# LuoGroup2023/PanTax

Hardware: AMD Instinct MI355X
Metric: PAO wall-time (s) + Mreads/s: packed reads + DB (graphs and their unique-trio index) resident in HBM -> abundance tables; the metric's own GAF -> abundance quantity is value_gaf_to_tables (files -> tables, never `value`) (higher is better)
Workload: dtype int64+f64

## Files before the change

### pantax_amd/csrc/cov_device.hpp

```cpp
#pragma once
#include "common.hpp"
#include "wave.hpp"

namespace ptx {

constexpr int COV_BLOCK = 256;

__device__ __forceinline__ uint32_t bm_peek(const uint32_t *p) {
    return __hip_atomic_load(p, __ATOMIC_RELAXED, __HIP_MEMORY_SCOPE_AGENT);
}
constexpr uint32_t COV_BWIN = 2048;
constexpr int COV_WIN = 2048;
extern __shared__ uint32_t s_cov[];
#define S_WIN(i) s_cov[(i)]
#define S_BM(bmo, i) s_cov[(bmo) + (i)]
#define S_FULL(bmo, i) reinterpret_cast<uint8_t *>(s_cov + (bmo) + COV_BWIN)[(i)]
__host__ __device__ constexpr size_t cov_lds_bytes(int win) { return (size_t)win * 4 + COV_BWIN * 4 + (size_t)win; }
__device__ __forceinline__ void lds_or(uint32_t *__restrict__ bm, uint32_t bmo, uint64_t bw0, uint32_t bwn, uint64_t w, uint32_t m) {
    const uint64_t off = w - bw0;
    if (off < bwn) {
        if ((S_BM(bmo, off) & m) != m) atomicOr(&S_BM(bmo, off), m);
    } else if ((bm_peek(&bm[w]) & m) != m) atomicOr(&bm[w], m);
}
__device__ __forceinline__ void mark_range(uint32_t *__restrict__ bm, uint32_t bmo, uint64_t bw0, uint32_t bwn, uint64_t g0, uint64_t g1) {
    if (g1 <= g0) return;
    uint64_t w0 = g0 >> 5, w1 = (g1 - 1) >> 5;
    uint32_t m0 = 0xFFFFFFFFu << (g0 & 31);
    uint32_t m1 = 0xFFFFFFFFu >> (31 - (uint32_t)((g1 - 1) & 31));
    if (w0 == w1) lds_or(bm, bmo, bw0, bwn, w0, m0 & m1);
    else {
        lds_or(bm, bmo, bw0, bwn, w0, m0);
        for (uint64_t w = w0 + 1; w < w1; ++w) lds_or(bm, bmo, bw0, bwn, w, 0xFFFFFFFFu);
        lds_or(bm, bmo, bw0, bwn, w1, m1);
    }
}
__device__ __forceinline__ void win_or(uint32_t bmo, uint32_t w, uint32_t m) { if ((S_BM(bmo, w) & m) != m) atomicOr(&S_BM(bmo, w), m); }
__device__ __forceinline__ void mark_window(uint32_t bmo, uint32_t r0, uint32_t r1) {
    if (r1 <= r0) return;
    const uint32_t w0 = r0 >> 5, w1 = (r1 - 1) >> 5;
    const uint32_t m0 = 0xFFFFFFFFu << (r0 & 31), m1 = 0xFFFFFFFFu >> (31 - ((r1 - 1) & 31));
    if (w0 == w1) win_or(bmo, w0, m0 & m1);
    else {
        win_or(bmo, w0, m0);
        for (uint32_t w = w0 + 1; w < w1; ++w) win_or(bmo, w, 0xFFFFFFFFu);
        win_or(bmo, w1, m1);
    }
}

constexpr uint32_t STEP_LONG = 0x80u;
constexpr uint32_t STEP_START = 0x40u, STEP_PAD = 0xFFu, STEP_DIST = 0x3Fu;
__device__ __forceinline__ unsigned long long ballot1(bool b) { return __builtin_amdgcn_ballot_w64(b); }
__device__ __forceinline__ bool any1(bool b) { return __builtin_amdgcn_ballot_w64(b) != 0ull; }
__device__ __forceinline__ bool none1(bool b) { return __builtin_amdgcn_ballot_w64(b) == 0ull; }
__device__ __forceinline__ uint32_t slot_in_group(uint32_t group_first_slot, uint32_t code, int lane) {
    const unsigned long long starts = ballot1((code != STEP_PAD) & ((code & STEP_START) != 0u)) & ~1ull;
    const uint32_t below = __builtin_amdgcn_mbcnt_hi((uint32_t)(starts >> 32), __builtin_amdgcn_mbcnt_lo((uint32_t)starts, 0u));
    return group_first_slot + below + (uint32_t)((starts >> lane) & 1ull);
}

__device__ __forceinline__ uint32_t rl_from_memory(uint32_t j, uint32_t b, const uint32_t *__restrict__ node_id, const uint8_t *__restrict__ step_dup,
                                                   uint32_t delta, const uint4 *__restrict__ node_rec, uint32_t len0, uint32_t ps) {
    const uint32_t idj = node_id[b + j];
    if (j == 0 || ((step_dup[b + j] & 1u) && idj == node_id[b])) return len0 - ps;
    return node_rec[idj + delta].z;
}

#ifdef COV_ABLATE
#define ABL(bit) (ablate & (bit))
#else
#define ABL(bit) false
#endif
constexpr int COV_WIN_BACK = 128;
constexpr uint32_t NO_SLOT = 0xFFFFFFFFu;

__device__ __forceinline__ void add_bases(unsigned long long *__restrict__ bases, uint32_t wlo, uint32_t win_n, uint32_t v, uint32_t aln) {
    const uint32_t off = v - wlo;
    if (off < win_n && aln < (1u << 18)) atomicAdd(&S_WIN(off), aln);
    else atomicAdd(&bases[v], (unsigned long long)aln);
}
constexpr uint32_t NO_FULL = 0xFFFFFFFFu;
__device__ __forceinline__ void mark_full_wave(uint32_t *__restrict__ full, uint32_t wlo, uint32_t win_n, uint32_t v) {
    const uint32_t off = v - wlo;
    const bool have = v != NO_FULL;
    if (have && off < win_n) S_FULL(COV_WIN, off) = 1;
    const bool out = have && off >= win_n;
    unsigned long long todo = __ballot(out);
    const uint32_t w = v >> 5, bit = 1u << (v & 31);
    const int lane = threadIdx.x & 63;
    while (todo) {
        const int leader = __builtin_ctzll(todo);
        const uint32_t wl = (uint32_t)__builtin_amdgcn_readlane((int)w, leader);
        const bool mine = out && w == wl;
        const uint32_t orv = wave_reduce(mine ? bit : 0u, [](uint32_t x, uint32_t y) { return x | y; });
        if (lane == leader) atomicOr(&full[wl], orv);
        todo &= ~__ballot(mine);
    }
}

constexpr uint32_t COV_ITEM_GROUPS = 128;
struct __attribute__((packed, aligned(4))) EntPair { uint32_t a, b, c, d; };
constexpr int COV_BLK_SHIFT = 11;

template <int WIN>
__device__ __forceinline__ void mark_full_out_wave(uint32_t *__restrict__ full, bool out, uint32_t v) {
    unsigned long long todo = ballot1(out);
    const uint32_t w = v >> 5, bit = 1u << (v & 31);
    const int lane = threadIdx.x & 63;
    while (todo) {
        const int leader = __builtin_ctzll(todo);
        const uint32_t wl = (uint32_t)__builtin_amdgcn_readlane((int)w, leader);
        const bool mine = out & (w == wl);
        const uint32_t orv = wave_reduce(mine ? bit : 0u, [](uint32_t x, uint32_t y) { return x | y; });
        if (lane == leader) atomicOr(&full[wl], orv);
        todo &= ~ballot1(mine);
    }
}

}
```

### pantax_amd/csrc/stage_cov.hip

```cpp
#include <chrono>
#include <cstdio>
#include <cstdlib>
#include "common.hpp"
#include "primitives.hpp"
#include "wave.hpp"
#include "cov_plan.hpp"
#include "cov_device.hpp"
#pragma clang diagnostic ignored "-Wbitwise-instead-of-logical"

namespace ptx {

template <bool WITH_TRIO, int U, int PASSES, int WIN, bool LONG = false>
#if !defined(COV_NO_PF3) && !defined(COV_NO_PF2) && !defined(COV_NO_PREFETCH)
__attribute__((amdgpu_waves_per_eu((U <= 2 && !LONG) ? 6 : 1)))
#endif
__global__ void __launch_bounds__(COV_BLOCK) coverage_fast_kernel(
    const uint2 *__restrict__ items, const uint32_t *__restrict__ group_slot, const uint4 *__restrict__ read_rec, const uint2 *__restrict__ slot_rec,
    const uint32_t *__restrict__ node_id, const uint8_t *__restrict__ step_code, const uint8_t *__restrict__ active,
    const uint4 *__restrict__ node_rec, const uint64_t *__restrict__ bit_off, uint64_t V, unsigned long long *__restrict__ bases,
    uint32_t *__restrict__ bitmap, uint32_t *__restrict__ full, const uint2 *__restrict__ trio_ent, unsigned long long *__restrict__ trio_bases,
    unsigned long long *__restrict__ n_abort, uint32_t ablate, int blk_shift,
    const uint32_t *__restrict__ long_sum = nullptr, const uint32_t *__restrict__ long_len0 = nullptr, uint32_t only_long = 0u,
    uint32_t chunk_groups = 0u, uint32_t total_groups = 0u, uint32_t win_back = 0u, const uint32_t *__restrict__ item_sel = nullptr,
    uint32_t spec_miss = 0u) {
    constexpr int WAVES = COV_BLOCK / 64;
#if !defined(COV_NO_PF3) && !defined(COV_NO_PF2) && !defined(COV_NO_PREFETCH)
    const int lane = threadIdx.x & 63, wave = LONG ? (int)(threadIdx.x >> 6) : __builtin_amdgcn_readfirstlane((int)(threadIdx.x >> 6));
#else
    const int lane = threadIdx.x & 63, wave = threadIdx.x >> 6;
#endif
    uint32_t g0, n_groups;
    if constexpr (LONG) { g0 = blockIdx.x * chunk_groups; n_groups = min(g0 + chunk_groups, total_groups); }
    else { const uint2 item = items[item_sel ? item_sel[blockIdx.x] : blockIdx.x]; g0 = item.x; n_groups = item.y; }
    for (int i = threadIdx.x; i < (int)(cov_lds_bytes(WIN) / 4); i += COV_BLOCK) s_cov[i] = 0;
    uint32_t wlo = 0, win_n = 0, mark_n = 0, bit0_lo = 0, bwn = 0;
    uint64_t bw0 = 0;
    uint32_t s0 = 0xFFFFFFFFu, dlt0 = 0;
#pragma unroll 1
    for (uint32_t g = g0; g < n_groups && win_n == 0; ++g) {
        const uint32_t gs = group_slot[g];
        if (gs == NO_SLOT) continue;
        const uint2 sr0 = slot_rec[gs];
        if ((int)sr0.x < 0 || !active[sr0.x]) continue;
        s0 = sr0.x; dlt0 = sr0.y;
        const uint32_t id0 = node_id[(uint64_t)g * 64], v0 = id0 + sr0.y, in_blk = id0 & ((1u << blk_shift) - 1u);
        const uint32_t back = LONG ? win_back : in_blk + 64u;
        wlo = (v0 > back ? v0 - back : 0u) & ~63u;
        win_n = WIN;
        const uint64_t b_lo = bit_off[wlo], b_hi = bit_off[min((uint64_t)wlo + WIN, V)];
        bw0 = b_lo >> 5;
        bit0_lo = (uint32_t)(bw0 << 5);
        bwn = COV_BWIN;
        mark_n = (b_hi - (bw0 << 5) <= (uint64_t)COV_BWIN * 32) ? (uint32_t)min((uint64_t)WIN, V - wlo) : 0u;
    }
    if (spec_miss) s0 = 0xFFFFFFFFu;
    __builtin_amdgcn_fence(__ATOMIC_RELEASE, "workgroup", "local");
    __builtin_amdgcn_s_barrier();
    __builtin_amdgcn_fence(__ATOMIC_ACQUIRE, "workgroup", "local");
#ifndef COV_NO_PREFETCH
    uint32_t n_code[U], n_id[U], n_gs[U];
    {
        const uint32_t gw0 = g0 + (uint32_t)(wave * U);
#pragma unroll
        for (int u = 0; u < U; ++u) {
            const uint32_t g = gw0 + (uint32_t)u < n_groups ? gw0 + (uint32_t)u : (gw0 < n_groups ? gw0 : g0);
            const uint64_t t = (uint64_t)g * 64 + lane;
            n_code[u] = step_code[t]; n_id[u] = node_id[t]; n_gs[u] = group_slot[g];
        }
    }
#endif
#if !defined(COV_NO_PF2) && !defined(COV_NO_PREFETCH)
    constexpr bool PF2 = !LONG;
#else
    constexpr bool PF2 = false;
#endif
#if !defined(COV_NO_PF3)
    constexpr bool PF3 = PF2;
#else
    constexpr bool PF3 = false;
#endif
    const auto guess_v = [&](uint32_t id) { const uint32_t vg = id + dlt0; return vg < V ? vg : wlo; };
    uint32_t c_code[U], c_id[U], c_gs[U];
    uint4 c_rr[U];
    uint2 c_sr[U];
    uint4 c_nr[U];
    bool c_run[U];
#pragma unroll
    for (int u = 0; u < U; ++u) c_run[u] = false;
    if constexpr (PF2) {
        const uint32_t gw0 = g0 + (uint32_t)(wave * U), gw1 = gw0 + (uint32_t)(WAVES * U);
#pragma unroll
        for (int u = 0; u < U; ++u) {
            c_code[u] = n_code[u]; c_id[u] = n_id[u]; c_gs[u] = n_gs[u];
            const uint32_t g = gw1 + (uint32_t)u < n_groups ? gw1 + (uint32_t)u : (gw0 < n_groups ? gw0 : g0);
            const uint64_t t = (uint64_t)g * 64 + lane;
            n_code[u] = step_code[t]; n_id[u] = node_id[t]; n_gs[u] = group_slot[g];
            const bool pad0 = c_code[u] == STEP_PAD;
            const bool run0 = (gw0 + (uint32_t)u < n_groups) & any1(!pad0) & none1(!pad0 & ((c_code[u] & STEP_LONG) != 0u));
            const uint32_t sl = slot_in_group(c_gs[u], c_code[u], lane);
            const uint32_t slot = (pad0 | !run0) ? (c_gs[u] == NO_SLOT ? 0u : c_gs[u]) : sl;
            c_rr[u] = read_rec[slot];
            if constexpr (PF3) c_sr[u] = make_uint2(slot_rec[slot].x, 0u); else c_sr[u] = slot_rec[slot];
            if constexpr (PF3) c_nr[u] = node_rec[guess_v(c_id[u])];
            c_run[u] = run0;
        }
        if constexpr (PF3) __builtin_amdgcn_sched_barrier(0);
    }
#pragma unroll 1
    for (int pass = 0;; ++pass) {
        const uint32_t gw = g0 + (uint32_t)((pass * WAVES + wave) * U);
        if (gw >= n_groups) break;
        uint32_t code[U], id[U], gs[U];
        bool run[U];
        uint4 rr[U];
        uint2 sr[U];
        uint4 nrg[U];
#ifndef COV_NO_PREFETCH
        if constexpr (PF2) {
            const uint32_t gn = gw + (uint32_t)(WAVES * U), g2 = gn + (uint32_t)(WAVES * U);
            uint32_t m_code[U], m_id[U], m_gs[U];
#pragma unroll
            for (int u = 0; u < U; ++u) {
                run[u] = c_run[u];
                code[u] = c_code[u]; id[u] = c_id[u]; gs[u] = c_gs[u]; rr[u] = c_rr[u]; sr[u] = c_sr[u];
                if constexpr (PF3) nrg[u] = c_nr[u];
                const uint32_t g = g2 + (uint32_t)u < n_groups ? g2 + (uint32_t)u : gw;
                const uint64_t t = (uint64_t)g * 64 + lane;
                m_code[u] = step_code[t]; m_id[u] = node_id[t]; m_gs[u] = group_slot[g];
                const bool padn = n_code[u] == STEP_PAD;
                const bool runn = (gn + (uint32_t)u < n_groups) & any1(!padn) & none1(!padn & ((n_code[u] & STEP_LONG) != 0u));
                const uint32_t sl = slot_in_group(n_gs[u], n_code[u], lane);
                const uint32_t slot = (padn | !runn) ? (n_gs[u] == NO_SLOT ? 0u : n_gs[u]) : sl;
                c_rr[u] = read_rec[slot];
                if constexpr (PF3) c_sr[u] = make_uint2(slot_rec[slot].x, 0u); else c_sr[u] = slot_rec[slot];
                if constexpr (PF3) c_nr[u] = node_rec[guess_v(n_id[u])];
                c_run[u] = runn;
                c_code[u] = n_code[u]; c_id[u] = n_id[u]; c_gs[u] = n_gs[u];
                n_code[u] = m_code[u]; n_id[u] = m_id[u]; n_gs[u] = m_gs[u];
            }
            if constexpr (PF3) __builtin_amdgcn_sched_barrier(0);
        } else
        {
            const uint32_t gn = gw + (uint32_t)(WAVES * U);
#pragma unroll
            for (int u = 0; u < U; ++u) {
                run[u] = gw + (uint32_t)u < n_groups;
                code[u] = n_code[u]; id[u] = n_id[u]; gs[u] = n_gs[u];
                const uint32_t g = gn + (uint32_t)u < n_groups ? gn + (uint32_t)u : gw;
                const uint64_t t = (uint64_t)g * 64 + lane;
                n_code[u] = step_code[t]; n_id[u] = node_id[t]; n_gs[u] = group_slot[g];
            }
        }
#else
#pragma unroll
        for (int u = 0; u < U; ++u) {
            const uint32_t g = gw + (uint32_t)u;
            run[u] = g < n_groups;
            const uint64_t t = (uint64_t)(run[u] ? g : gw) * 64 + lane;
            code[u] = step_code[t]; id[u] = node_id[t];
            gs[u] = group_slot[run[u] ? g : gw];
        }
#endif
        bool pad[U];
        uint32_t slot_[U];
        uint32_t ll0[U], lsum[U];
#pragma unroll
        for (int u = 0; u < U; ++u) {
            pad[u] = code[u] == STEP_PAD;
            if constexpr (!PF2) {
                const bool has_long = any1(!pad[u] & ((code[u] & STEP_LONG) != 0u));
                run[u] = run[u] & any1(!pad[u]) & (LONG ? (has_long | (only_long == 0u)) : !has_long);
            }
            const uint32_t sl = slot_in_group(gs[u], code[u], lane);
            const uint32_t slot = (pad[u] | !run[u]) ? (gs[u] == NO_SLOT ? 0u : gs[u]) : sl;
            if constexpr (!PF2) { rr[u] = read_rec[slot]; sr[u] = slot_rec[slot]; }
            if constexpr (LONG) { ll0[u] = long_len0[slot]; lsum[u] = long_sum[slot]; }
            slot_[u] = slot;
        }
        uint32_t h_id1[U], h_id2[U], h_codes[U];
        if constexpr (LONG) {
#pragma unroll
            for (int u = 0; u < U; ++u) {
                const uint32_t gu = (uint32_t)__builtin_amdgcn_readfirstlane((int)(gw + (uint32_t)u));
                const uint64_t t0 = (uint64_t)(run[u] && gu != 0u ? gu : 1u) * 64;
                h_id1[u] = node_id[t0 - 1]; h_id2[u] = node_id[t0 - 2];
                h_codes[u] = *reinterpret_cast<const uint32_t *>(step_code + t0 - 4);
            }
        }
        uint4 nr[U];
        uint32_t v[U], act[U];
        bool ok[U];
#pragma unroll
        for (int u = 0; u < U; ++u) {
            ok[u] = run[u] & !pad[u] & ((int)sr[u].x >= 0);
            if constexpr (PF3) {
                if (none1(ok[u] & (sr[u].x != s0))) {
                    v[u] = ok[u] ? id[u] + dlt0 : wlo;
                    nr[u] = nrg[u];
                    asm volatile("" : "+v"(nr[u].x), "+v"(nr[u].y), "+v"(nr[u].z), "+v"(nr[u].w));
                } else {
                    v[u] = ok[u] ? id[u] + slot_rec[slot_[u]].y : wlo;
                    nr[u] = node_rec[v[u]];
                    const uint32_t a = active[ok[u] ? sr[u].x : 0u];
                    asm volatile("" : "+v"(nr[u].x), "+v"(nr[u].y), "+v"(nr[u].z), "+v"(nr[u].w));
                    ok[u] = ok[u] & (a != 0u);
                }
                act[u] = 1u;
            } else {
            v[u] = ok[u] ? id[u] + sr[u].y : wlo;
            nr[u] = node_rec[v[u]];
            act[u] = active[ok[u] ? sr[u].x : 0u];
            }
        }
        uint32_t idf[U], i0_[U], hv1[U], hv2[U];
        uint4 nrh1[U], nrh2[U];
        if constexpr (LONG) {
#pragma unroll
            for (int u = 0; u < U; ++u) {
                idf[u] = node_id[rr[u].x];
                const uint32_t gbase = (gw + (uint32_t)u) * 64u;
                const bool ok0 = __builtin_amdgcn_readfirstlane((int)ok[u]) != 0;
                i0_[u] = ok0 ? (uint32_t)__builtin_amdgcn_readfirstlane((int)(gbase - rr[u].x)) : 0u;
                const uint32_t delta0 = (uint32_t)__builtin_amdgcn_readfirstlane((int)sr[u].y);
                hv1[u] = i0_[u] >= 1u ? h_id1[u] + delta0 : wlo;
                hv2[u] = i0_[u] >= 2u ? h_id2[u] + delta0 : wlo;
                nrh1[u] = node_rec[hv1[u]]; nrh2[u] = node_rec[hv2[u]];
            }
        }
        uint32_t i_[U], nl[U], len0[U], nh[U], hx[U], tlo[U], thi[U];
        uint2 e0[U], e1[U];
        bool live[U], single[U], dead_read[U], cross[U];
        int dist[U];
#pragma unroll
        for (int u = 0; u < U; ++u) {
            const uint32_t gbase = (gw + (uint32_t)u) * 64u;
            i_[u] = gbase + (uint32_t)lane - rr[u].x;
            ok[u] = ok[u] & (act[u] != 0u);
            nl[u] = ok[u] ? nr[u].z : 0u;
            if constexpr (LONG) {
                dist[u] = (int)min(ok[u] ? i_[u] : 0u, (uint32_t)lane);
                cross[u] = ok[u] & (i_[u] > (uint32_t)lane);
                const uint32_t in_wave = __shfl(nl[u], lane - dist[u]);
                len0[u] = cross[u] ? ll0[u] : in_wave;
            } else
            len0[u] = __shfl(nl[u], lane - (int)i_[u]);
            uint32_t v2 = wave_shr1(wave_shr1(v[u]));
            uint32_t hw1 = wave_shr1(nr[u].w), hy1 = wave_shr1(nr[u].y);
            if constexpr (LONG) {
                v2 = lane == 0 ? hv2[u] : lane == 1 ? hv1[u] : v2;
                hw1 = lane == 0 ? nrh1[u].w : hw1; hy1 = lane == 0 ? nrh1[u].y : hy1;
            }
            single[u] = rr[u].y == 1u;
            dead_read[u] = !single[u] & (rr[u].z > len0[u]);
            live[u] = ok[u] & !dead_read[u] & !(single[u] & (rr[u].w < rr[u].z));
            nh[u] = 0; hx[u] = 0; tlo[u] = 0; thi[u] = 0;
            e0[u] = make_uint2(0u, 0u); e1[u] = e0[u];
            if (WITH_TRIO && !ABL(4u)) {
                hx[u] = hw1;
                tlo[u] = min(v[u], v2); thi[u] = max(v[u], v2);
                nh[u] = (live[u] & (i_[u] >= 2u) & ((nr_filter(hy1) & nr_pair_bit(tlo[u], thi[u])) != 0u)) ? nr_rows(hy1) : 0u;
                const EntPair ep = *reinterpret_cast<const EntPair *>(trio_ent + (nh[u] ? hx[u] : 0u));
                e0[u] = make_uint2(ep.a, ep.b); e1[u] = make_uint2(ep.c, ep.d);
            }
        }
#pragma unroll
        for (int u = 0; u < U; ++u) {
            const uint32_t k = rr[u].y, ps = rr[u].z, pe = rr[u].w, i = i_[u];
            if (any1(ok[u] & dead_read[u] & (i == 0u))) { if (ok[u] & dead_read[u] & (i == 0u)) atomicAdd(n_abort, 1ull); }
            const uint32_t contrib = (live[u] & !single[u]) ? (i == 0u ? nl[u] - ps : nl[u]) : 0u;
            const uint32_t pexcl = wave_incl_scan_dpp(contrib) - contrib;
            uint32_t seen = pexcl - __shfl(pexcl, lane - (LONG ? dist[u] : (int)i));
            if constexpr (LONG) seen = cross[u] ? lsum[u] - ps : seen;
            const uint32_t tgt = pe - ps;
            uint32_t aln = nl[u];
            if (i + 1u == k) aln = ((pe >= ps) & (tgt > seen)) ? tgt - seen : 0u;
            if (i == 0u) aln = single[u] ? tgt : nl[u] - ps;
            const uint32_t sidx = i == 0u ? ps : 0u;
            uint32_t hi = sidx + aln;
            if (hi > nl[u]) hi = nl[u];
            const bool markable = live[u] & (hi > sidx) & !(single[u] & !((ps < pe) & (pe <= nl[u])));
            const uint32_t dupd = code[u] & STEP_DIST;
            bool earlier = dupd != 0u, at_step0 = dupd == i;
            if constexpr (LONG) {
                const bool lc = (code[u] & STEP_LONG) != 0u;
                const uint32_t id_first = cross[u] ? idf[u] : __shfl(id[u], lane - dist[u]);
                earlier = lc ? (code[u] & 1u) != 0u : earlier;
                at_step0 = lc ? id[u] == id_first : at_step0;
            }
            const uint32_t rl = !live[u] ? 0u : !earlier ? aln : (at_step0 ? len0[u] - ps : nl[u]);
            const uint32_t off = v[u] - wlo;
            const bool inw = off < win_n;
            if (live[u] & !earlier & (aln != 0u) && !ABL(2u)) {
                if (inw & (aln < (1u << 18))) atomicAdd(&S_WIN(off), aln);
                else atomicAdd(&bases[v[u]], (unsigned long long)aln);
            }
            const bool whole = markable & (sidx == 0u) & (hi == nl[u]);
            if constexpr (LONG) { if (!ABL(1u) && !ABL(8u)) mark_full_out_wave<WIN>(full, whole & !inw, v[u]); }
            if (markable && !ABL(1u)) {
                if (whole) {
                    if (inw) S_FULL(WIN, off) = 1; else if (!LONG && !ABL(8u)) atomicOr(&full[v[u] >> 5], 1u << (v[u] & 31));
                } else if (off < mark_n) {
                    const uint32_t rel = nr[u].x - bit0_lo;
                    mark_window(WIN, rel + sidx, rel + hi);
                } else if (!ABL(8u)) {
                    const uint64_t bo = nr_bit_off(nr[u]);
                    mark_range(bitmap, WIN, bw0, bwn, bo + sidx, bo + hi);
                }
            }
            if (WITH_TRIO && !ABL(4u)) {
                uint32_t rl1 = wave_shr1(rl), rl2 = wave_shr1(rl1);
                if constexpr (LONG) {
                    const uint32_t idf0 = (uint32_t)__builtin_amdgcn_readfirstlane((int)idf[u]), l0 = (uint32_t)__builtin_amdgcn_readfirstlane((int)len0[u]),
                                   ps0 = (uint32_t)__builtin_amdgcn_readfirstlane((int)ps);
                    const uint32_t c1 = h_codes[u] >> 24, c2 = (h_codes[u] >> 16) & 0xFFu;
                    const uint32_t rlh1 = ((i0_[u] == 1u) | (((c1 & 1u) != 0u) & (h_id1[u] == idf0))) ? l0 - ps0 : nrh1[u].z;
                    const uint32_t rlh2 = ((i0_[u] == 2u) | (((c2 & 1u) != 0u) & (h_id2[u] == idf0))) ? l0 - ps0 : nrh2[u].z;
                    rl2 = lane == 0 ? rlh2 : lane == 1 ? rlh1 : rl2;
                    rl1 = lane == 0 ? rlh1 : rl1;
                }
                constexpr uint32_t NO_ROW = 0xFFFFFFFFu;
                const bool m0 = (nh[u] != 0u) & (e0[u].x == tlo[u]) & (e0[u].y == thi[u]);
                const bool m1 = (nh[u] > 1u) & (e1[u].x == tlo[u]) & (e1[u].y == thi[u]);
                uint32_t row = m0 ? hx[u] : m1 ? hx[u] + 1u : NO_ROW;
                if (any1(!(m0 | m1) & (nh[u] > 2u))) {
                    if (!(m0 | m1) & (nh[u] > 2u))
                        for (uint32_t j = 2; j < nh[u]; ++j) {
                            const uint2 e = trio_ent[hx[u] + j];
                            if (e.x == tlo[u] && e.y == thi[u]) { row = hx[u] + j; break; }
                        }
                }
                const uint32_t sum = rl2 + rl1 + rl;
                if ((row != NO_ROW) & (sum != 0u)) atomicAdd(&trio_bases[row], (unsigned long long)sum);
            }
        }
    }
    __syncthreads();
    if (win_n) {
        for (int i = threadIdx.x; i < WIN; i += COV_BLOCK) {
            const uint32_t c = S_WIN(i);
            if (c) atomicAdd(&bases[wlo + i], (unsigned long long)c);
            const unsigned long long fb = __ballot(S_FULL(WIN, i) != 0);
            if (fb && (lane & 31) == 0 && !ABL(32u)) {
                const uint32_t m = (uint32_t)(fb >> (lane & 32));
                if (m) atomicOr(&full[(wlo + i) >> 5], m);
            }
        }
        if (!ABL(16u))
        for (uint32_t i = threadIdx.x; i < bwn; i += COV_BLOCK) {
            const uint32_t m = S_BM(WIN, i);
            if (m) atomicOr(&bitmap[bw0 + i], m);
        }
    }
}

template <int WS_U, bool EAGER = false>
__global__ void __launch_bounds__(256) walk_sum_kernel(uint64_t T, const uint32_t *__restrict__ group_slot, const uint8_t *__restrict__ step_dup,
                                                       const uint4 *__restrict__ read_rec, const uint2 *__restrict__ slot_rec,
                                                       const uint32_t *__restrict__ node_id, const uint32_t *__restrict__ node_len,
                                                       uint32_t *__restrict__ long_sum, uint32_t *__restrict__ long_len0) {
    const int lane = threadIdx.x & 63;
    const uint64_t stride = (uint64_t)gridDim.x * 256 * WS_U;
    for (uint64_t base = ((uint64_t)blockIdx.x * 256 + (threadIdx.x - lane)) * WS_U; base < T; base += stride) {
        uint32_t code[WS_U], slot[WS_U], id[WS_U], nl[WS_U], gs_e[WS_U], id_e[WS_U];
        uint64_t t[WS_U];
        bool any = false;
#pragma unroll
        for (int u = 0; u < WS_U; ++u) {
            t[u] = base + (uint64_t)u * 64 + lane;
            code[u] = t[u] < T ? step_dup[t[u]] : STEP_PAD;
            if constexpr (EAGER) { gs_e[u] = t[u] < T ? group_slot[t[u] >> 6] : NO_SLOT; id_e[u] = t[u] < T ? node_id[t[u]] : 0u; }
        }
#pragma unroll
        for (int u = 0; u < WS_U; ++u) any = any || (code[u] != STEP_PAD && (code[u] & STEP_LONG));
        if (!__any(any)) continue;
#pragma unroll
        for (int u = 0; u < WS_U; ++u) {
            slot[u] = NO_SLOT; id[u] = 0;
            uint32_t gs;
            if constexpr (EAGER) gs = gs_e[u]; else gs = t[u] < T ? group_slot[t[u] >> 6] : NO_SLOT;
            const uint32_t sl = slot_in_group(gs, code[u], lane);
            if (code[u] != STEP_PAD && (code[u] & STEP_LONG)) { slot[u] = sl; if constexpr (EAGER) id[u] = id_e[u]; else id[u] = node_id[t[u]]; }
        }
        uint2 sr[WS_U];
        uint4 rr[WS_U];
#pragma unroll
        for (int u = 0; u < WS_U; ++u) {
            sr[u] = make_uint2(0xFFFFFFFFu, 0u); rr[u] = make_uint4(0u, 0u, 0u, 0u);
            if (slot[u] != NO_SLOT) { sr[u] = slot_rec[slot[u]]; rr[u] = read_rec[slot[u]]; }
        }
#pragma unroll
        for (int u = 0; u < WS_U; ++u) {
            nl[u] = 0;
            const bool counted = slot[u] != NO_SLOT && (int)sr[u].x >= 0 && (uint32_t)(t[u] - rr[u].x) + 1 < rr[u].y;
            if (counted) nl[u] = node_len[id[u] + sr[u].y];
        }
#pragma unroll
        for (int u = 0; u < WS_U; ++u) {
            if (!__any(slot[u] != NO_SLOT)) continue;
            if (slot[u] != NO_SLOT && (int)sr[u].x >= 0 && (uint32_t)(t[u] - rr[u].x) + 1 < rr[u].y && t[u] == rr[u].x)
                long_len0[slot[u]] = nl[u];
            const uint32_t prev = __shfl_up(slot[u], 1);
            const bool head = lane == 0 || prev != slot[u];
            const unsigned long long heads = __ballot(head);
            const int start = 63 - __builtin_clzll(heads & ((2ull << lane) - 1ull));
            const uint32_t sc = wave_incl_scan_dpp(nl[u]);
            const uint32_t front = __shfl(sc, start > 0 ? start - 1 : 0);
            const uint32_t incl = sc - (start > 0 ? front : 0u);
            const unsigned long long after = heads & ~((2ull << lane) - 1ull);
            const bool tail = after ? (lane + 1 == __builtin_ctzll(after)) : lane == 63;
            if (tail && slot[u] != NO_SLOT && incl) atomicAdd(&long_sum[slot[u]], incl);
        }
    }
}

__global__ void __launch_bounds__(256) popcount_kernel(uint64_t V, const uint64_t *__restrict__ bit_off, const uint32_t *__restrict__ full,
                                                       const uint32_t *__restrict__ bitmap, uint32_t *__restrict__ cov) {
    for (uint64_t v = (uint64_t)blockIdx.x * 256 + threadIdx.x; v < V; v += (uint64_t)gridDim.x * 256) {
        uint64_t g0 = bit_off[v], g1 = bit_off[v + 1];
        uint32_t c = 0;
        if ((full[v >> 5] >> (uint32_t)(v & 31)) & 1u) c = (uint32_t)(g1 - g0);
        else if (g1 > g0) {
            uint64_t w0 = g0 >> 5, w1 = (g1 - 1) >> 5;
            uint32_t m0 = 0xFFFFFFFFu << (g0 & 31);
            uint32_t m1 = 0xFFFFFFFFu >> (31 - (uint32_t)((g1 - 1) & 31));
            if (w0 == w1) c = __popc(bitmap[w0] & m0 & m1);
            else {
                c = __popc(bitmap[w0] & m0);
                for (uint64_t w = w0 + 1; w < w1; ++w) c += __popc(bitmap[w]);
                c += __popc(bitmap[w1] & m1);
            }
        }
        cov[v] = c;
    }
}

constexpr uint32_t PCL_WORDS = 2304;
__global__ void __launch_bounds__(256) popcount_long_kernel(uint64_t V, const uint64_t *__restrict__ bit_off, const uint32_t *__restrict__ full,
                                                            const uint32_t *__restrict__ bitmap, uint32_t *__restrict__ cov) {
    __shared__ __attribute__((aligned(16))) uint32_t s_prefix[4 * PCL_WORDS];
    const uint32_t lane = threadIdx.x & 63, wave = threadIdx.x >> 6;
    uint32_t *pw = s_prefix + wave * PCL_WORDS;
    const uint64_t n_str = (V + 63) / 64;
    for (uint64_t st = (uint64_t)blockIdx.x * 4 + wave; st < n_str; st += (uint64_t)gridDim.x * 4) {
        const uint64_t v = st * 64 + lane;
        const bool in = v < V;
        const uint64_t g0 = in ? bit_off[v] : 0ull, g1 = in ? bit_off[v + 1] : 0ull;
        const uint64_t b0 = __shfl(g0, 0);
        const uint32_t last = (uint32_t)min((uint64_t)63, V - 1 - st * 64);
        const uint64_t b1 = __shfl(g1, (int)last);
        const uint64_t wa = (b0 >> 5) & ~3ull, nw = b1 > b0 ? ((b1 - 1) >> 5) - wa + 1 : 0;
        const bool coop = nw <= (uint64_t)PCL_WORDS && __builtin_amdgcn_ballot_w64(in && g1 - g0 > 64ull) != 0ull;
        if (coop) {
            uint32_t carry = 0;
            for (uint32_t k = 0; k < (uint32_t)nw; k += 256) {
                const uint32_t i = k + 4u * lane;
                const uint4 x = i < (uint32_t)nw ? *reinterpret_cast<const uint4 *>(bitmap + wa + i) : make_uint4(0u, 0u, 0u, 0u);
                const uint32_t p0 = (uint32_t)__popc(x.x), p1 = p0 + (uint32_t)__popc(x.y), p2 = p1 + (uint32_t)__popc(x.z), p3 = p2 + (uint32_t)__popc(x.w);
                const uint32_t incl = wave_incl_scan_dpp(p3);
                const uint32_t base = carry + incl - p3;
                if (i < (uint32_t)nw) *reinterpret_cast<uint4 *>(pw + i) = make_uint4(base, base + p0, base + p1, base + p2);
                carry += (uint32_t)__builtin_amdgcn_readlane((int)incl, 63);
            }
            __builtin_amdgcn_fence(__ATOMIC_RELEASE, "workgroup", "local");
            __builtin_amdgcn_wave_barrier();
            __builtin_amdgcn_fence(__ATOMIC_ACQUIRE, "workgroup", "local");
        }
        uint32_t c = 0;
        if (in && g1 > g0) {
            const uint64_t w0 = g0 >> 5, w1 = (g1 - 1) >> 5;
            const uint32_t m0 = 0xFFFFFFFFu << (g0 & 31), m1 = 0xFFFFFFFFu >> (31 - (uint32_t)((g1 - 1) & 31));
            if ((full[v >> 5] >> (uint32_t)(v & 31)) & 1u) c = (uint32_t)(g1 - g0);
            else if (coop) c = (pw[w1 - wa] + (uint32_t)__popc(bitmap[w1] & m1)) - (pw[w0 - wa] + (uint32_t)__popc(bitmap[w0] & ~m0));
            else if (w0 == w1) c = __popc(bitmap[w0] & m0 & m1);
            else {
                c = __popc(bitmap[w0] & m0);
                for (uint64_t w = w0 + 1; w < w1; ++w) c += __popc(bitmap[w]);
                c += __popc(bitmap[w1] & m1);
            }
        }
        if (coop) __builtin_amdgcn_wave_barrier();
        if (in) cov[v] = c;
    }
}

__global__ void __launch_bounds__(256) count_nonzero_words_kernel(const uint32_t *__restrict__ p, uint64_t n, unsigned long long *__restrict__ out) {
    unsigned long long c = 0;
    for (uint64_t i = (uint64_t)blockIdx.x * 256 + threadIdx.x; i < n; i += (uint64_t)gridDim.x * 256) c += p[i] != 0u;
    if (c) atomicAdd(out, c);
}

int coverage_prepare(Ctx *ctx, Db *db, Reads *rd, bool with_trio) {
    const CovArenaLayout a = cov_arena_layout(db->V, with_trio ? db->U : 0, db->L);
    const size_t off_trio = a.off_trio, off_bm = a.off_bm, off_full = a.off_full, total = a.total;
    PTX_HIP(ctx, db->d_cov_arena.alloc(total));
    uint8_t *base = db->d_cov_arena.p;
    db->d_bases.view(base, db->V);
    db->d_trio_bases.view(base + off_trio, a.n_trio);
    db->d_abort = reinterpret_cast<unsigned long long *>(base + a.off_abort);
    db->d_bitmap.view(base + off_bm, a.words);
    db->d_full.view(base + off_full, a.fwords);
    const uint64_t sig = (uint64_t)(uintptr_t)base ^ ((uint64_t)total * 0x9E3779B97F4A7C15ull) ^ ((uint64_t)off_bm << 1) ^ ((uint64_t)off_full << 2) ^ (uint64_t)off_trio;
    db->cov_arena_total = total;
    if (db->cov_clean_pending) {
        PTX_HIP(ctx, hipStreamWaitEvent(ctx->stream, db->ev_cov_clean, 0));
        db->cov_clean_pending = false;
    }
    if (db->cov_arena_clean && db->cov_arena_sig == sig) {
        if (ctx->cfg.cov_arena_verify) {
            DevBuf<unsigned long long> d_nz;
            PTX_HIP(ctx, d_nz.alloc(1));
            PTX_HIP(ctx, hipMemsetAsync(d_nz.p, 0, 8, ctx->stream));
            PTX_HIP(ctx, hipMemsetAsync(db->d_abort, 0, 8, ctx->stream));
            hipLaunchKernelGGL(count_nonzero_words_kernel, dim3(grid_for(total / 4, 256, ctx->n_cu * 8)), dim3(256), 0, ctx->stream, reinterpret_cast<const uint32_t *>(base), (uint64_t)(total / 4), d_nz.p);
            unsigned long long nz = 0;
            PTX_TRY(download(ctx, &nz, d_nz.p, 1));
            PTX_HIP(ctx, hipStreamSynchronize(ctx->stream));
            if (nz) return fail(ctx, PANTAX_HIP_E_STATE, "coverage_prepare: %llu non-zero words in an arena its last readers should have left clean", nz);
        }
        PTX_HIP(ctx, hipMemsetAsync(db->d_abort, 0, 8, ctx->stream));
    } else {
        KTimer t(ctx, "zero_fill_kernel");
        PTX_TRY(zero_fill(ctx, base, total));
    }
    db->cov_arena_clean = false;
    db->cov_arena_sig = sig;
    if (rd->R && rd->T_pad && rd->n_long && rd->long_sums_db != 0 && rd->long_sums_db == db->uid) {
    } else if (rd->R && rd->T_pad && rd->n_long) {
        PTX_HIP(ctx, hipMemsetAsync(rd->d_long_sum.p, 0, rd->R * sizeof(uint32_t), ctx->stream));
        KTimer t(ctx, "walk_sum_kernel");
        const bool eager = (uint64_t)rd->n_long * 2 > rd->n_slots;
        hipLaunchKernelGGL((eager ? walk_sum_kernel<4, true> : walk_sum_kernel<4, false>), dim3(grid_for(rd->T_pad / 4 + 1, 256, ctx->n_cu * 16)), dim3(256), 0, ctx->stream, rd->T_pad, rd->d_g_group_slot.p,
                           rd->d_g_step_dup.p, rd->d_g_read_rec.p, rd->d_g_slot_rec.p, rd->d_g_node_id.p, db->d_node_len.p, rd->d_long_sum.p,
                           rd->d_long_len0.p);
    }
    PTX_HIP(ctx, hipGetLastError());
    db->cov_prepared = true;
    return 0;
}

int coverage_arena_clean_async(Ctx *ctx, Db *db) {
    if (!db->d_cov_arena.p || !db->cov_arena_total || !ctx->stream2) return 0;
    uint8_t *f_ptr = db->d_cov_arena.p;
    const size_t f_n = db->cov_arena_total;
    if (!db->ev_cov_read) PTX_HIP(ctx, hipEventCreateWithFlags(&db->ev_cov_read, hipEventDisableTiming));
    if (!db->ev_cov_clean) PTX_HIP(ctx, hipEventCreateWithFlags(&db->ev_cov_clean, hipEventDisableTiming));
    PTX_HIP(ctx, hipEventRecord(db->ev_cov_read, ctx->stream));
    PTX_HIP(ctx, hipStreamWaitEvent(ctx->stream2, db->ev_cov_read, 0));
    hipStream_t main_stream = ctx->stream;
    ctx->stream_main = main_stream; ctx->stream = ctx->stream2;
    int rc;
    rc = zero_fill(ctx, f_ptr, f_n);
    const hipError_t e = hipEventRecord(db->ev_cov_clean, ctx->stream2);
    ctx->stream = main_stream; ctx->stream_main = nullptr;
    if (rc != 0) return rc;
    PTX_HIP(ctx, e);
    db->cov_done = false;
    db->cov_arena_clean = true; db->cov_clean_pending = true;
    return 0;
}

struct CovLap {
    Ctx *ctx;
    bool on;
    std::chrono::steady_clock::time_point prev = std::chrono::steady_clock::now();
    void operator()(const char *what) {
        if (!on) return;
        (void)hipStreamSynchronize(ctx->stream);
        const auto now = std::chrono::steady_clock::now();
        std::fprintf(stderr, "[node_coverage]        %-28s %9.3f ms\n", what, std::chrono::duration<double, std::milli>(now - prev).count());
        prev = now;
    }
};

static int active_flags(Ctx *ctx, Db *db, const uint8_t *d_active, const uint8_t **out) {
    if (!d_active) {
        if (db->d_ones.n < db->S) { PTX_HIP(ctx, db->d_ones.alloc(db->S)); PTX_HIP(ctx, hipMemsetAsync(db->d_ones.p, 1, db->S, ctx->stream)); }
        d_active = db->d_ones.p;
    }
    *out = d_active;
    return 0;
}

struct ItemList { uint32_t n; const uint32_t *d; };
static int item_selection(Ctx *ctx, Db *db, const Reads *rd, ItemList *out) {
    *out = {rd->n_items, nullptr};
    if (db->item_sel_layout == rd->layout_id && rd->layout_id != 0) {
        *out = {db->item_sel_n, db->item_sel_on ? db->d_item_sel.p : nullptr};
    } else if (rd->h_item_block.size() == rd->n_items && rd->item_blk_shift > 0 && db->S && !db->h_range_start.empty()) {
        const CovItemSel s = cov_item_select(rd->h_item_block, rd->item_blk_shift, db->h_range_start, db->h_range_end);
        if (s.on && s.n_sel) PTX_TRY(upload(ctx, db->d_item_sel, s.sel.data(), s.sel.size()));
        *out = {s.n_sel, s.on && s.n_sel ? db->d_item_sel.p : nullptr};
        db->item_sel_layout = rd->layout_id; db->item_sel_n = s.n_sel; db->item_sel_on = s.on;
    }
    return 0;
}

struct CovFastTail {
    const uint2 *items; int blk_shift; const uint32_t *long_sum, *long_len0; uint32_t only_long, chunk_groups, total_groups, win_back; const uint32_t *item_sel;
};
template <int U, int PASSES, int WIN, bool LONG>
static void fast_launch_as(Ctx *ctx, Db *db, Reads *rd, const uint8_t *d_act, bool trio, int grid, const CovFastTail &t) {
    if (grid <= 0) return;
    const auto kernel = trio ? coverage_fast_kernel<true, U, PASSES, WIN, LONG> : coverage_fast_kernel<false, U, PASSES, WIN, LONG>;
    hipLaunchKernelGGL(kernel, dim3(grid), dim3(COV_BLOCK), cov_lds_bytes(WIN), ctx->stream, t.items, rd->d_g_group_slot.p, rd->d_g_read_rec.p,
                       rd->d_g_slot_rec.p, rd->d_g_node_id.p, rd->d_g_step_dup.p, d_act, db->d_node_rec.p, db->d_bit_off.p, db->V, db->d_bases.p,
                       db->d_bitmap.p, db->d_full.p, db->d_trio_ent.p, db->d_trio_bases.p, db->d_abort, ctx->cfg.cov_ablate ,
                       t.blk_shift, t.long_sum, t.long_len0, t.only_long, t.chunk_groups, t.total_groups, t.win_back, t.item_sel,
                       ctx->cfg.cov_spec == "miss" ? 1u : 0u );
}

static int fast_launch(Ctx *ctx, Db *db, Reads *rd, const uint8_t *d_act, bool trio, const CovFastShape &f, const ItemList &list) {
    const CovFastTail t{rd->d_g_items.p, rd->item_blk_shift, nullptr, nullptr, 0u, 0u, 0u, 0u, list.d};
    const int grid = (int)list.n;
    const auto is = [&](int u, int passes, int win) { return f.u == u && f.passes == passes && f.win == win; };
    if (is(1, 8, 2048)) fast_launch_as<1, 8, 2048, false>(ctx, db, rd, d_act, trio, grid, t);
    else if (is(2, 4, 2048)) fast_launch_as<2, 4, 2048, false>(ctx, db, rd, d_act, trio, grid, t);
    else if (is(2, 8, 2048)) fast_launch_as<2, 8, 2048, false>(ctx, db, rd, d_act, trio, grid, t);
    else if (is(2, 8, 3072)) fast_launch_as<2, 8, 3072, false>(ctx, db, rd, d_act, trio, grid, t);
    else if (is(2, 8, 4096)) fast_launch_as<2, 8, 4096, false>(ctx, db, rd, d_act, trio, grid, t);
    else if (is(2, 4, 3072)) fast_launch_as<2, 4, 3072, false>(ctx, db, rd, d_act, trio, grid, t);
    else if (is(2, 8, 2304)) fast_launch_as<2, 8, 2304, false>(ctx, db, rd, d_act, trio, grid, t);
    else if (is(2, 8, 2560)) fast_launch_as<2, 8, 2560, false>(ctx, db, rd, d_act, trio, grid, t);
    else if (is(2, 4, 2304)) fast_launch_as<2, 4, 2304, false>(ctx, db, rd, d_act, trio, grid, t);
    else if (is(2, 4, 2560)) fast_launch_as<2, 4, 2560, false>(ctx, db, rd, d_act, trio, grid, t);
    else if (is(1, 8, 2304)) fast_launch_as<1, 8, 2304, false>(ctx, db, rd, d_act, trio, grid, t);
    else if (is(4, 4, 2304)) fast_launch_as<4, 4, 2304, false>(ctx, db, rd, d_act, trio, grid, t);
    else if (is(4, 4, 2048)) fast_launch_as<4, 4, 2048, false>(ctx, db, rd, d_act, trio, grid, t);
    else if (is(4, 4, 3072)) fast_launch_as<4, 4, 3072, false>(ctx, db, rd, d_act, trio, grid, t);
    else return fail(ctx, PANTAX_HIP_E_STATE, "coverage_launch: no short-read kernel of shape U = %d, PASSES = %d, WIN = %d", f.u, f.passes, f.win);
    return 0;
}

static int long_launch(Ctx *ctx, Db *db, Reads *rd, const uint8_t *d_act, bool trio, const CovPlan &plan) {
    if (!rd->d_long_sum.p) { PTX_HIP(ctx, rd->d_long_sum.alloc(rd->R)); PTX_HIP(ctx, rd->d_long_len0.alloc(rd->R)); }
    const CovLongShape &l = plan.lng;
    const uint32_t total_groups = (uint32_t)(rd->T_pad / 64);
    const int grid = (int)((total_groups + l.chunk_groups - 1) / l.chunk_groups);
    const CovFastTail t{nullptr, 0, rd->d_long_sum.p, rd->d_long_len0.p, plan.only_long ? 1u : 0u, l.chunk_groups, total_groups, l.win_back, nullptr};
    if (l.u == 1 && l.win == 2048) fast_launch_as<1, 1, 2048, true>(ctx, db, rd, d_act, trio, grid, t);
    else if (l.u == 1 && l.win == 3072) fast_launch_as<1, 1, 3072, true>(ctx, db, rd, d_act, trio, grid, t);
    else if (l.u == 1 && l.win == 4096) fast_launch_as<1, 1, 4096, true>(ctx, db, rd, d_act, trio, grid, t);
    else if (l.u == 2 && l.win == 2048) fast_launch_as<2, 1, 2048, true>(ctx, db, rd, d_act, trio, grid, t);
    else if (l.u == 2 && l.win == 4096) fast_launch_as<2, 1, 4096, true>(ctx, db, rd, d_act, trio, grid, t);
    else if (l.u == 2 && l.win == 3072) fast_launch_as<2, 1, 3072, true>(ctx, db, rd, d_act, trio, grid, t);
    else return fail(ctx, PANTAX_HIP_E_STATE, "coverage_launch: no long-walk kernel of shape U = %d, WIN = %d", l.u, l.win);
    return 0;
}

static int count_launch(Ctx *ctx, Db *db) {
    PTX_HIP(ctx, db->d_cov.alloc(db->V));
    KTimer t(ctx, "popcount_kernel");
    if (long_node_shape(db->L, db->V, ctx->cfg.ncs_prefix_min, ctx->cfg.ncs_no_prefix))
        hipLaunchKernelGGL(popcount_long_kernel, dim3(grid_for((db->V + 63) / 64, 4, ctx->n_cu * 8)), dim3(256), 0, ctx->stream, db->V,
                           db->d_bit_off.p, db->d_full.p, db->d_bitmap.p, db->d_cov.p);
    else
        hipLaunchKernelGGL(popcount_kernel, dim3(grid_for(db->V, 256, ctx->n_cu * 8)), dim3(256), 0, ctx->stream, db->V,
                           db->d_bit_off.p, db->d_full.p, db->d_bitmap.p, db->d_cov.p);
    return 0;
}

int coverage_launch(Ctx *ctx, Db *db, Reads *rd, const uint8_t *d_active, bool with_trio, bool defer_count) {
    if (!rd->grouped) return fail(ctx, PANTAX_HIP_E_STATE, "node_coverage: these reads are a slice kept as plain columns (to be routed to their owner), not resident reads");
    const bool trace = ctx->cfg.trace && !defer_count;
    CovLap lap{ctx, trace};
    if (!db->cov_prepared) PTX_TRY(coverage_prepare(ctx, db, rd, with_trio));
    lap("arena + zero fill");
    db->cov_prepared = false;
    db->cov_stage = false;
    db->trio_free_valid = false;
    const bool trio = with_trio && db->U;
    const uint8_t *d_act_fast = d_active;
    if (rd->R && rd->T_pad) PTX_TRY(active_flags(ctx, db, d_active, &d_act_fast));
    const CtxConfig &cfg = ctx->cfg;
    const CovPlan plan = cov_plan(rd->T_pad, rd->n_long, rd->n_slots, rd->n_items, rd->R, cfg.cov_general, cfg.cov_long, cfg.covf_shape, cfg.covl_shape,
                                  cfg.cov_shape, cfg.cov_xcd);
    if (plan.run_fast) {
        KTimer t(ctx, "coverage_fast_kernel");
        ItemList list;
        PTX_TRY(item_selection(ctx, db, rd, &list));
        if (trace) std::fprintf(stderr, "[node_coverage]        %u of %u items launched\n", list.n, rd->n_items);
        PTX_TRY(fast_launch(ctx, db, rd, d_act_fast, trio, plan.fast, list));
    }
    if (plan.run_long) {
        KTimer t(ctx, "coverage_long_kernel");
        PTX_TRY(long_launch(ctx, db, rd, d_act_fast, trio, plan));
    }
    if (plan.run_step) {
        KTimer t(ctx, "coverage_step_kernel");
        PTX_TRY(coverage_step_launch(ctx, db, rd, d_active, trio, plan));
    }
    PTX_HIP(ctx, hipGetLastError());
    lap("coverage kernels");
    db->cov_count_pending = defer_count && db->V != 0;
    if (db->V && !defer_count) PTX_TRY(count_launch(ctx, db));
    PTX_HIP(ctx, hipGetLastError());
    lap("popcount");
    db->cov_done = true;
    return 0;
}

}
```

Before: 7341.

## Make coverage kernel LDS updates branch-free using per-lane dummy slots

For non-long groups, the coverage kernel now performs its window base adds, full-node flags and partial bitmap marks unconditionally. Inactive lanes are redirected to per-lane dummy LDS slots, added by enlarging the shared-memory allocation, so divergent branches disappear and the abort counting becomes one popcounted ballot. The slot computation is also moved out of the PF3 path into the later lane-dependent code, and the LDS flush index is tied to wave and lane. The cost is extra unconditional LDS atomics on lanes that have nothing to write, more shared memory per block, and a one-off bitmap path that still keeps a global fallback branch.

```diff
diff --git a/pantax_amd/csrc/cov_device.hpp b/pantax_amd/csrc/cov_device.hpp
--- a/pantax_amd/csrc/cov_device.hpp
+++ b/pantax_amd/csrc/cov_device.hpp
@@ -15,7 +15,11 @@
 #define S_WIN(i) s_cov[(i)]
 #define S_BM(bmo, i) s_cov[(bmo) + (i)]
 #define S_FULL(bmo, i) reinterpret_cast<uint8_t *>(s_cov + (bmo) + COV_BWIN)[(i)]
-__host__ __device__ constexpr size_t cov_lds_bytes(int win) { return (size_t)win * 4 + COV_BWIN * 4 + (size_t)win; }
+constexpr uint32_t COV_DUMMY = 64;
+__host__ __device__ constexpr size_t cov_lds_bytes(int win) { return (size_t)win * 4 + COV_BWIN * 4 + (size_t)win + COV_DUMMY * 9; }
+__host__ __device__ constexpr uint32_t cov_dummy_win(int win) { return (uint32_t)win + COV_BWIN + (uint32_t)win / 4u; }
+__host__ __device__ constexpr uint32_t cov_dummy_bm(int win) { return COV_BWIN + (uint32_t)win / 4u + COV_DUMMY; }
+__host__ __device__ constexpr uint32_t cov_dummy_full(int win) { return (uint32_t)win + COV_DUMMY * 8u; }
 __device__ __forceinline__ void lds_or(uint32_t *__restrict__ bm, uint32_t bmo, uint64_t bw0, uint32_t bwn, uint64_t w, uint32_t m) {
     const uint64_t off = w - bw0;
     if (off < bwn) {
@@ -47,11 +51,25 @@
     }
 }
 
+__device__ __forceinline__ void mark_window_flat(uint32_t bmo, bool on, uint32_t r0, uint32_t r1, uint32_t dummy) {
+    const uint32_t w0 = on ? r0 >> 5 : dummy, w1 = on ? (r1 - 1u) >> 5 : dummy;
+    const uint32_t m0 = 0xFFFFFFFFu << (r0 & 31), m1 = 0xFFFFFFFFu >> (31 - ((r1 - 1u) & 31));
+    const uint32_t span = w1 - w0;
+    const uint32_t first = span != 0u ? m0 : m0 & m1;
+    atomicOr(&S_BM(bmo, w0), on ? first : 0u);
+    atomicOr(&S_BM(bmo, w1), span != 0u ? m1 : 0u);
+    if (__builtin_amdgcn_ballot_w64(span > 1u) != 0ull) {
+        if (span > 1u)
+            for (uint32_t w = w0 + 1u; w < w1; ++w) atomicOr(&S_BM(bmo, w), 0xFFFFFFFFu);
+    }
+}
+
 constexpr uint32_t STEP_LONG = 0x80u;
 constexpr uint32_t STEP_START = 0x40u, STEP_PAD = 0xFFu, STEP_DIST = 0x3Fu;
 __device__ __forceinline__ unsigned long long ballot1(bool b) { return __builtin_amdgcn_ballot_w64(b); }
 __device__ __forceinline__ bool any1(bool b) { return __builtin_amdgcn_ballot_w64(b) != 0ull; }
 __device__ __forceinline__ bool none1(bool b) { return __builtin_amdgcn_ballot_w64(b) == 0ull; }
+__device__ __forceinline__ bool long_step(uint32_t code) { return code - STEP_LONG < STEP_PAD - STEP_LONG; }
 __device__ __forceinline__ uint32_t slot_in_group(uint32_t group_first_slot, uint32_t code, int lane) {
     const unsigned long long starts = ballot1((code != STEP_PAD) & ((code & STEP_START) != 0u)) & ~1ull;
     const uint32_t below = __builtin_amdgcn_mbcnt_hi((uint32_t)(starts >> 32), __builtin_amdgcn_mbcnt_lo((uint32_t)starts, 0u));
diff --git a/pantax_amd/csrc/stage_cov.hip b/pantax_amd/csrc/stage_cov.hip
--- a/pantax_amd/csrc/stage_cov.hip
+++ b/pantax_amd/csrc/stage_cov.hip
@@ -79,6 +79,11 @@
 #else
     constexpr bool PF3 = false;
 #endif
+#if !defined(COV_R26_BODY)
+    constexpr bool FLAT = !LONG;
+#else
+    constexpr bool FLAT = false;
+#endif
     const auto guess_v = [&](uint32_t id) { const uint32_t vg = id + dlt0; return vg < V ? vg : wlo; };
     uint32_t c_code[U], c_id[U], c_gs[U];
     uint4 c_rr[U];
@@ -96,7 +101,7 @@
             const uint64_t t = (uint64_t)g * 64 + lane;
             n_code[u] = step_code[t]; n_id[u] = node_id[t]; n_gs[u] = group_slot[g];
             const bool pad0 = c_code[u] == STEP_PAD;
-            const bool run0 = (gw0 + (uint32_t)u < n_groups) & any1(!pad0) & none1(!pad0 & ((c_code[u] & STEP_LONG) != 0u));
+            const bool run0 = (gw0 + (uint32_t)u < n_groups) & any1(!pad0) & none1(long_step(c_code[u]));
             const uint32_t sl = slot_in_group(c_gs[u], c_code[u], lane);
             const uint32_t slot = (pad0 | !run0) ? (c_gs[u] == NO_SLOT ? 0u : c_gs[u]) : sl;
             c_rr[u] = read_rec[slot];
@@ -128,7 +133,7 @@
                 const uint64_t t = (uint64_t)g * 64 + lane;
                 m_code[u] = step_code[t]; m_id[u] = node_id[t]; m_gs[u] = group_slot[g];
                 const bool padn = n_code[u] == STEP_PAD;
-                const bool runn = (gn + (uint32_t)u < n_groups) & any1(!padn) & none1(!padn & ((n_code[u] & STEP_LONG) != 0u));
+                const bool runn = (gn + (uint32_t)u < n_groups) & any1(!padn) & none1(long_step(n_code[u]));
                 const uint32_t sl = slot_in_group(n_gs[u], n_code[u], lane);
                 const uint32_t slot = (padn | !runn) ? (n_gs[u] == NO_SLOT ? 0u : n_gs[u]) : sl;
                 c_rr[u] = read_rec[slot];
@@ -171,11 +176,13 @@
                 const bool has_long = any1(!pad[u] & ((code[u] & STEP_LONG) != 0u));
                 run[u] = run[u] & any1(!pad[u]) & (LONG ? (has_long | (only_long == 0u)) : !has_long);
             }
+            if constexpr (!PF3) {
             const uint32_t sl = slot_in_group(gs[u], code[u], lane);
             const uint32_t slot = (pad[u] | !run[u]) ? (gs[u] == NO_SLOT ? 0u : gs[u]) : sl;
             if constexpr (!PF2) { rr[u] = read_rec[slot]; sr[u] = slot_rec[slot]; }
             if constexpr (LONG) { ll0[u] = long_len0[slot]; lsum[u] = long_sum[slot]; }
             slot_[u] = slot;
+            }
         }
         uint32_t h_id1[U], h_id2[U], h_codes[U];
         if constexpr (LONG) {
@@ -199,6 +206,8 @@
                     nr[u] = nrg[u];
                     asm volatile("" : "+v"(nr[u].x), "+v"(nr[u].y), "+v"(nr[u].z), "+v"(nr[u].w));
                 } else {
+                    const uint32_t sl = slot_in_group(gs[u], code[u], lane);
+                    slot_[u] = (pad[u] | !run[u]) ? (gs[u] == NO_SLOT ? 0u : gs[u]) : sl;
                     v[u] = ok[u] ? id[u] + slot_rec[slot_[u]].y : wlo;
                     nr[u] = node_rec[v[u]];
                     const uint32_t a = active[ok[u] ? sr[u].x : 0u];
@@ -229,7 +238,7 @@
         }
         uint32_t i_[U], nl[U], len0[U], nh[U], hx[U], tlo[U], thi[U];
         uint2 e0[U], e1[U];
-        bool live[U], single[U], dead_read[U], cross[U];
+        bool live[U], single[U], dead_read[U], cross[U], abrt[U];
         int dist[U];
 #pragma unroll
         for (int u = 0; u < U; ++u) {
@@ -253,6 +262,7 @@
             single[u] = rr[u].y == 1u;
             dead_read[u] = !single[u] & (rr[u].z > len0[u]);
             live[u] = ok[u] & !dead_read[u] & !(single[u] & (rr[u].w < rr[u].z));
+            abrt[u] = ok[u] & dead_read[u] & (i_[u] == 0u);
             nh[u] = 0; hx[u] = 0; tlo[u] = 0; thi[u] = 0;
             e0[u] = make_uint2(0u, 0u); e1[u] = e0[u];
             if (WITH_TRIO && !ABL(4u)) {
@@ -266,7 +276,7 @@
 #pragma unroll
         for (int u = 0; u < U; ++u) {
             const uint32_t k = rr[u].y, ps = rr[u].z, pe = rr[u].w, i = i_[u];
-            if (any1(ok[u] & dead_read[u] & (i == 0u))) { if (ok[u] & dead_read[u] & (i == 0u)) atomicAdd(n_abort, 1ull); }
+            if constexpr (!FLAT) { if (any1(abrt[u])) { if (abrt[u]) atomicAdd(n_abort, 1ull); } }
             const uint32_t contrib = (live[u] & !single[u]) ? (i == 0u ? nl[u] - ps : nl[u]) : 0u;
             const uint32_t pexcl = wave_incl_scan_dpp(contrib) - contrib;
             uint32_t seen = pexcl - __shfl(pexcl, lane - (LONG ? dist[u] : (int)i));
@@ -290,6 +300,31 @@
             const uint32_t rl = !live[u] ? 0u : !earlier ? aln : (at_step0 ? len0[u] - ps : nl[u]);
             const uint32_t off = v[u] - wlo;
             const bool inw = off < win_n;
+            if constexpr (FLAT) {
+                const uint32_t a = (live[u] & !earlier & !ABL(2u)) ? aln : 0u;
+                const bool add_l = inw & (a - 1u < (1u << 18) - 1u);
+                const uint32_t a_l = add_l ? a : 0u, a_g = a - a_l;
+                atomicAdd(&S_WIN(add_l ? off : cov_dummy_win(WIN) + (uint32_t)lane), a_l);
+                const bool mk = markable & !ABL(1u);
+                const bool whole = (sidx == 0u) & (hi == nl[u]);
+                const bool full_l = mk & whole & inw, part_l = mk & !whole & (off < mark_n);
+                S_FULL(WIN, full_l ? off : cov_dummy_full(WIN) + (uint32_t)lane) = 1;
+                const uint32_t rel = nr[u].x - bit0_lo;
+                mark_window_flat(WIN, part_l, rel + sidx, rel + hi, cov_dummy_bm(WIN) + (uint32_t)lane);
+                const bool mark_g = mk & !(full_l | part_l) & !ABL(8u);
+                if (any1((a_g != 0u) | mark_g | abrt[u])) {
+                    const unsigned long long ab = ballot1(abrt[u]);
+                    if ((ab != 0ull) & (lane == 0)) atomicAdd(n_abort, (unsigned long long)__builtin_popcountll(ab));
+                    if (a_g != 0u) atomicAdd(&bases[v[u]], (unsigned long long)a_g);
+                    if (mark_g) {
+                        if (whole) atomicOr(&full[v[u] >> 5], 1u << (v[u] & 31));
+                        else {
+                            const uint64_t bo = nr_bit_off(nr[u]);
+                            mark_range(bitmap, WIN, bw0, bwn, bo + sidx, bo + hi);
+                        }
+                    }
+                }
+            } else {
             if (live[u] & !earlier & (aln != 0u) && !ABL(2u)) {
                 if (inw & (aln < (1u << 18))) atomicAdd(&S_WIN(off), aln);
                 else atomicAdd(&bases[v[u]], (unsigned long long)aln);
@@ -306,6 +341,7 @@
                     const uint64_t bo = nr_bit_off(nr[u]);
                     mark_range(bitmap, WIN, bw0, bwn, bo + sidx, bo + hi);
                 }
+            }
             }
             if (WITH_TRIO && !ABL(4u)) {
                 uint32_t rl1 = wave_shr1(rl), rl2 = wave_shr1(rl1);
@@ -335,8 +371,9 @@
         }
     }
     __syncthreads();
+    const int tid = PF3 ? wave * 64 + lane : (int)threadIdx.x;
     if (win_n) {
-        for (int i = threadIdx.x; i < WIN; i += COV_BLOCK) {
+        for (int i = tid; i < WIN; i += COV_BLOCK) {
             const uint32_t c = S_WIN(i);
             if (c) atomicAdd(&bases[wlo + i], (unsigned long long)c);
             const unsigned long long fb = __ballot(S_FULL(WIN, i) != 0);
@@ -346,7 +383,7 @@
             }
         }
         if (!ABL(16u))
-        for (uint32_t i = threadIdx.x; i < bwn; i += COV_BLOCK) {
+        for (uint32_t i = (uint32_t)tid; i < bwn; i += COV_BLOCK) {
             const uint32_t m = S_BM(WIN, i);
             if (m) atomicOr(&bitmap[bw0 + i], m);
         }
```

Result: no change. 7301 (-0.5%).
